# SpaceLearner/SessionRec-pytorch

Hardware: AMD Instinct MI355X
Metric: sessions/sec training, Yoochoose-1/64 batch 512 (higher is better)
Workload: dtype bf16 (MFMA operands; fp32 accumulate, master weights, scoring); 1 GPU; MSGIFSR training step, synthetic Yoochoose-1/64 shape (V=37484 items, d=256, batch 512 per GPU, session length<=20, order 3, dropout 0.1); global_batch=512, parallelism=single GPU

## Files before the change

include/srec.h:

```cpp
#ifndef SREC_H
#define SREC_H
#include "srec_hg.h"

#ifdef __cplusplus
extern "C" {
#endif

#define SREC_BAD_ARG 1001

int srec_gemm_f32(const float* A, int a_rs, int a_cs, const float* B, int b_rs, int b_cs, float* C, int ldc,
                  const float* bias, int M, int N, int K, const int* dyn, int dyn_mode, float alpha, float beta,
                  float* ws, long ws_floats, void* stream);

int srec_gemm_bf16_nt(const float* A, int lda, const float* B, int ldb, float* C, int ldc, const float* bias, int M,
                      int N, int K, const int* dyn, float alpha, float beta, float* ws, long ws_floats, void* stream);

int srec_gemm_bf16_tn(const float* A, int lda, const float* B, int ldb, float* C, int ldc, int Mred, int N, int K,
                      const int* dyn, float alpha, float beta, float* ws, long ws_floats, void* stream);

int srec_ce_plan(int B, int V, int d, int* n_item_tiles, int* n_ranges);
int srec_score_ce_fwd(const float* sr, int ld_sr, const float* E, int ld_e, const float* cs, const int* labels,
                      int B, int V, int d, const int* dynB, float* ws_stats, float* lab_logit, float* lse,
                      float* lossvec, float* loss, void* stream);
int srec_score_ce_bwd(const float* sr, int ld_sr, const float* E, int ld_e, const float* cs, const int* labels,
// ... 173 lines not shown
                          const float* part, const int* cptr, int u_cap, int n_part, void* stream);
int srec_adam_rows_multi(float* W, const float* G, float* M, float* V, int n, int d, int ld, const float* hyper, int use_wd,
                         float max_norm, int renorm_write, float* cs_out, float cs_scale, int eps_mode, float cs_eps,
                         const float* proj_cs, float proj_inv_scale, float* radial, void* dst16, int Dp, int* slot,
                         const float* part, const int* cptr, int u_cap, int n_part, const void* desc, const float* multi_hyper,
                         void* stream);

int srec_hg_ws_floats(const void* desc, long* n_floats);
int srec_hg_fwd(const void* desc, const float* x, int ld_x, float* out, int ld_out, unsigned char* arg, void* stream);
int srec_hg_fold(const void* desc, void* stream);
int srec_step_prep(const void* desc, void* stream);
int srec_hg_drop_prep(const float* x, const float* cnt, int rows, int D, float p, int seed, const int* counter, int salt,
                      float* ms, float* xc, float* rm, float* xres, float pa, long na, float* mk, void* stream);
int srec_hg_drop_prep16(const float* x, const float* cnt, int rows, int D, float p, int seed, const int* counter, int salt,
                        float* ms, float* xc, float* rm, float* xres, float pa, long na, float* mk, void* xc16, void* stream);
int srec_hg_drop_merge(const float* t, int S, const float* ms, long n, float* dx, float p, int seed, const int* counter,
                       int salt, void* stream);
int srec_hg_pre_merge(const void* desc, const float* g, int ld_g, const float* t, int S, float* dx, int ld_dx, void* stream);
int srec_hg_bwd(const void* desc, const float* x, int ld_x, const float* g, int ld_g, const unsigned char* arg, float* dx,
                int ld_dx, float* ws, void* stream);

int srec_gemm_group_bf16(const void* desc, int mode, void* stream);

int srec_gemm_f32_group_run(const void* desc, float* ws, long ws_floats, void* stream);
int srec_gemm_f32_group_run_defer(const void* desc, float* ws, long ws_floats, long* slab_off, int* slab_n, void* stream);
int srec_gemm16_nt(const void* desc, void* stream);
int srec_gemm16_tn(const void* desc, void* stream);
int srec_rows_bf16(const float* src, int ld, int n, const int* dyn, int d, void* dst16, void* stream);
int srec_sum_slabs(const float* part, int C, int R, long n, float* out, void* stream);
int srec_weights_bf16(int n, const void* W, const void* W16, const void* WT16, const int* R, const int* Cc, void* stream);
int srec_norm_perm_pick_fwd(const float* x, int ld_x, const int* perm, int n_cap, const int* dyn_t, int D, int eps_mode,
                            float eps, float* allf, float* invr, int npick, int B, const int* dyn_b, const void* pick,
                            const void* pout, const int* ld_p, void* stream);
int srec_norm_perm_pick_bwd(const float* allf, const float* invr, const float* g_allf, int ld_g, const int* perm, int n_cap,
                            const int* cat_seg, int B, const int* dyn_b, int D, int npick, const void* pick, const void* g_pick,
                            const int* ld_gp, float* dx, int ld_dx, int nt, const int* row0, const int* ncap, const void* dyn_n,
                            int n_rows, void* stream);
int srec_gru_step_fwd(const void* desc, void* stream);
int srec_gru_step_bwd(const void* desc, void* stream);
int srec_gru_fused_fwd(const void* desc, void* stream);
int srec_gru_wfrag(int n, const void* W, const void* dst, int d, void* stream);
// ... 64 lines not shown
```

sessionrec-pytorch_amd/csrc/gemm16.hip:

```cpp
#include "common.h"
#include "../../include/srec_hg.h"

namespace {

typedef __bf16 bf16x8 __attribute__((ext_vector_type(8)));
typedef short short2_t __attribute__((ext_vector_type(2)));
constexpr int G16_MAXP = 16, G16_MAXS = 4;

struct G16Args {
    const unsigned short* A[G16_MAXP][G16_MAXS];
    const unsigned short* B[G16_MAXP][G16_MAXS];
    void* C[G16_MAXP];
    const int* dyn[G16_MAXP];
    int M[G16_MAXP], N[G16_MAXP], K[G16_MAXP], nseg[G16_MAXP], koff[G16_MAXP], nsplit[G16_MAXP], start[G16_MAXP + 1];
    int np, lda, ldb, ldc;
    int ldap[G16_MAXP], ldbp[G16_MAXP], ldcp[G16_MAXP];
    float beta;
    int keep_dead;
    int per_xcd;
    int xcd_gs;
};

__device__ __forceinline__ unsigned lds_addr(const void* p) {
    return (unsigned)(size_t)(__attribute__((address_space(3))) const void*)p;
}

__device__ __forceinline__ void glds16(const unsigned short* sbase, unsigned voff, unsigned lds_dst) {
    unsigned keep;
// ... 21 lines not shown
    else if (PDV >= 3 && ahead >= 2) wait_vm<2 * IPS>();
    else if (PDV >= 2 && ahead >= 1) wait_vm<IPS>();
    else wait_vm<0>();
}

#ifdef SREC_G16_TIMING
__device__ unsigned long long g_g16_tim[8];
__device__ unsigned long long g_g16_blk[8192][2];
#define G16T(i) do { __builtin_amdgcn_sched_barrier(0); g16t[i] = __builtin_readcyclecounter(); __builtin_amdgcn_sched_barrier(0); } while (0)
#else
#define G16T(i)
#endif

constexpr int NS = 4, PD = 3;

template <int TM, int TN, bool C16, int BK = 32, int NS = 4, int NW = 4>
__global__ __launch_bounds__(64 * NW) void gemm16_nt_kernel(G16Args g) {
    constexpr int WN = NW / 2, NT = 64 * NW;
    constexpr int PD = NS - 1;
    constexpr int RPI = 512 / BK;
    constexpr int PPR = BK / 8;
    constexpr int FS = BK == 32 ? 2 : 1;
    constexpr int IM = TM / 64, IN = TN / (32 * WN);
    constexpr int STG = (TM + TN) * BK;
    constexpr int NIA = TM / RPI, NI = (TM + TN) / RPI;
    constexpr int IPS = NI / NW;
    static_assert(NI % NW == 0, "every wave must issue the same number of DMA instructions per stage");
    extern __shared__ __attribute__((aligned(16))) unsigned short smem[];

    const int bid = xcd_tile(g);
    if (bid >= g.start[g.np]) return;
#ifdef SREC_G16_TIMING
// ... 16 lines not shown
    unsigned short* __restrict__ C16p = static_cast<unsigned short*>(g.C[p]);
    if (m0 >= Ml) {
        if (!g.keep_dead && (C16 || g.beta == 0.f))
            for (int i = tid; i < TM * TN / 4; i += NT) {
                const int r = m0 + (i * 4) / TN, c = n0 + (i * 4) % TN;
                if (r < M && c + 3 < N) {
                    if (C16) *reinterpret_cast<uint2*>(C16p + (size_t)r * g.ldcp[p] + c) = make_uint2(0u, 0u);
                    else *reinterpret_cast<float4*>(C + (size_t)r * g.ldcp[p] + c) = make_float4(0.f, 0.f, 0.f, 0.f);
                } else if (r < M) {
                    for (int e = 0; e < 4; ++e)
                        if (c + e < N) { if (C16) C16p[(size_t)r * g.ldcp[p] + c + e] = 0; else C[(size_t)r * g.ldcp[p] + c + e] = 0.f; }
                }
            }
        return;
    }

    f32x16 acc[IM][IN];
#pragma unroll
    for (int i = 0; i < IM; ++i)
#pragma unroll
        for (int j = 0; j < IN; ++j)
#pragma unroll
            for (int r = 0; r < 16; ++r) acc[i][j][r] = 0.f;

    const int nk = K / BK, total = nk * g.nseg[p];
    const unsigned lds0 = lds_addr(smem);
    const int rl = lane / PPR, sl = lane % PPR;
    unsigned voff[IPS];
#pragma unroll
    for (int ii = 0; ii < IPS; ++ii) {
        const int i = ii * NW + wave;
        const int r = RPI * (i < NIA ? i : i - NIA) + rl;
        const unsigned pc = (unsigned)((sl ^ ((r >> FS) & (PPR - 1))) * 8);
        voff[ii] = i < NIA ? ((unsigned)min(r, Ml - 1 - m0) * (unsigned)g.ldap[p] + pc) * 2u
                           : ((unsigned)min(r, N - 1 - n0) * (unsigned)g.ldbp[p] + pc) * 2u;
    }
    int is_seg = 0, is_k = 0;
    const unsigned short* Aseg = g.A[p][0] + (size_t)m0 * g.ldap[p];
    const unsigned short* Bseg = g.B[p][0] + (size_t)n0 * g.ldbp[p];
    auto stage = [&](int it) {
        const unsigned dst = lds0 + (unsigned)((it % NS) * STG) * 2u;
#pragma unroll
        for (int ii = 0; ii < IPS; ++ii) {
            const int i = ii * NW + wave;
            glds16((i < NIA ? Aseg : Bseg) + is_k, voff[ii], dst + (unsigned)i * 1024u);
        }
        is_k += BK;
        if (is_k >= K) {
            is_k = 0;
            if (++is_seg < g.nseg[p]) {
                Aseg = g.A[p][is_seg] + (size_t)m0 * g.ldap[p];
                Bseg = g.B[p][is_seg] + (size_t)n0 * g.ldbp[p];
            }
        }
    };

    for (int s = 0; s < PD && s < total; ++s) stage(s);
    G16T(1);
    for (int it = 0; it < total; ++it) {
        G16T(2);
        wait_stage<IPS, PD>(min(total - it - 1, PD - 1));
        __syncthreads();
        G16T(3);
        if (it + PD < total) stage(it + PD);
        G16T(4);
        const unsigned short* As = smem + (it % NS) * STG;
// ... 32 lines not shown
#pragma unroll
        for (int i = 0; i < IM; ++i)
#pragma unroll
            for (int j = 0; j < IN; ++j)
#pragma unroll
                for (int q = 0; q < 4; ++q) {
                    uint2 v;
                    v.x = srec_pack_bf16(acc[i][j][4 * q], acc[i][j][4 * q + 1]);
                    v.y = srec_pack_bf16(acc[i][j][4 * q + 2], acc[i][j][4 * q + 3]);
                    *reinterpret_cast<uint2*>(patch + (i * 32 + l31) * LDP + j * 32 + 8 * q + 4 * half) = v;
                }
        constexpr int PPW = WC / 8;
#pragma unroll
        for (int t = 0; t < WR * PPW / 64; ++t) {
            const int idx = t * 64 + lane, rr = idx / PPW, pc = idx % PPW;
            const int row = m0 + wm * WR + rr, col = n0 + wn * WC + pc * 8;
            if (row >= M || (g.keep_dead && row >= Ml)) continue;
            uint4 v = *reinterpret_cast<const uint4*>(patch + rr * LDP + pc * 8);
            if (row >= Ml) v = make_uint4(0u, 0u, 0u, 0u);
            if (col + 7 < N) {
                *reinterpret_cast<uint4*>(C16p + (size_t)row * g.ldcp[p] + col) = v;
            } else {
                const unsigned short* e = reinterpret_cast<const unsigned short*>(&v);
                for (int k = 0; k < 8; ++k)
                    if (col + k < N) C16p[(size_t)row * g.ldcp[p] + col + k] = e[k];
            }
        }
#ifdef SREC_G16_TIMING
        asm volatile("s_waitcnt vmcnt(0)" ::: "memory");
        G16T(7);
        if (threadIdx.x == 0 && bid < 8192) g_g16_blk[bid][1] = __builtin_amdgcn_s_memrealtime();
        if (threadIdx.x == 0 && bid == 17) { g_g16_tim[0] = g16t[1] - g16t[0]; g_g16_tim[1] = g16w; g_g16_tim[2] = g16d; g_g16_tim[3] = g16c; g_g16_tim[4] = g16t[7] - g16t[6]; g_g16_tim[5] = g16t[7] - g16t[0]; g_g16_tim[6] = total; }
#endif
        return;
// ... 261 lines not shown
        }
        g.start[p] = blocks;
        blocks += cdiv(d->M[p], tm) * cdiv(d->N[p], tn) * g.nsplit[p];
    }
    g.start[d->np] = blocks;
    return 0;
}

template <typename K>
int optin(K kernel, int bytes, std::atomic<unsigned long long>& done) {
    return bytes > 64 * 1024 ? srec_lds_optin((const void*)kernel, bytes, done) : 0;
}

}

extern "C" int srec_gemm16_nt(const void* desc_, void* stream) {
    const srec_gemm16_group* h = (const srec_gemm16_group*)desc_;
    if (h == nullptr || h->np <= 0 || h->np > G16_MAXP) return SREC_BAD_ARG;
    G16Args g{};
    int blocks = 0;
    auto Mh = [&](int p) { return (h->mhint[p] > 0 && h->mhint[p] < h->M[p]) ? h->mhint[p] : h->M[p]; };
    long t128 = 0, rows_cap = 0, rows_live = 0;
    for (int p = 0; p < h->np; ++p) { t128 += (long)cdiv(Mh(p), 128) * cdiv(h->N[p], 128); rows_cap += h->M[p]; rows_live += Mh(p); }
    int nmax = 0;
    for (int p = 0; p < h->np; ++p) nmax = h->N[p] > nmax ? h->N[p] : nmax;
    int tm = (t128 >= 384 && nmax > 256) ? 128 : 64;
    long t64x128 = 0;
    for (int p = 0; p < h->np; ++p) t64x128 += (long)cdiv(Mh(p), 64) * cdiv(h->N[p], 128);
    if (!(h->c16 & SREC_G16_C_BF16) && tm == 64 && t64x128 > 384) {
        const long r64 = cdiv((int)cdiv((int)t64x128, 8), 96), r128 = cdiv((int)cdiv((int)t128, 8), 64);
        if (r128 * 105 < r64 * 100 || (r128 <= r64 && t128 >= 256)) tm = 128;
    }
    const int tn = (tm == 64 && t64x128 < 192) ? 64 : 128;
    if (int rc = fill(g, desc_, tm, tn, false, blocks)) return rc;
    if (!(h->c16 & SREC_G16_C_BF16)) {
        bool same_tn = true;
        const int tn0 = cdiv(h->N[0], tn);
        for (int p = 1; p < h->np; ++p) same_tn = same_tn && cdiv(h->N[p], tn) == tn0;
        if (same_tn && rows_live * 10 < rows_cap * 9) {
            g.xcd_gs = tn0;
            blocks = cdiv(blocks, 8 * tn0) * 8 * tn0;
        } else {
            g.per_xcd = cdiv(blocks, 8); blocks = 8 * g.per_xcd;
        }
    }
    hipStream_t st = (hipStream_t)stream;
    const bool c16 = h->c16 & SREC_G16_C_BF16;
    static std::atomic<unsigned long long> optin_mask[8];
#define SREC_G16(TMV, TNV, C16V, BKV, NSV, slot)                                                                       \
    do {                                                                                                               \
        const size_t lds = (size_t)NSV * (TMV + TNV) * BKV * 2;                                                        \
        if (int rc = optin(gemm16_nt_kernel<TMV, TNV, C16V, BKV, NSV>, (int)lds, optin_mask[slot])) return rc;         \
        hipLaunchKernelGGL((gemm16_nt_kernel<TMV, TNV, C16V, BKV, NSV>), dim3(blocks), dim3(256), lds, st, g);         \
    } while (0)
    const bool deep = blocks <= 384;
    if (tn == 64) {
        if (c16) SREC_G16(64, 64, true, 64, 2, 0); else if (deep) SREC_G16(64, 64, false, 64, 4, 1); else SREC_G16(64, 64, false, 64, 2, 2);
    } else if (deep && tm == 64 && !c16) {
        SREC_G16(64, 128, false, 64, 4, 3);
    } else if (tm == 128) {
        if (c16) SREC_G16(128, 128, true, 32, 3, 4); else SREC_G16(128, 128, false, 64, 2, 5);
    } else {
        if (c16) SREC_G16(64, 128, true, 32, 3, 6); else SREC_G16(64, 128, false, 64, 2, 7);
    }
#undef SREC_G16
    SREC_LAUNCH_CHECK();
    return 0;
}

#ifdef SREC_G16_TIMING
extern "C" int srec_g16_timing(unsigned long long* tim8, unsigned long long* blk) {
    if (hipMemcpyFromSymbol(tim8, HIP_SYMBOL(g_g16_tim), sizeof(unsigned long long) * 8) != hipSuccess) return 1;
    return hipMemcpyFromSymbol(blk, HIP_SYMBOL(g_g16_blk), sizeof(unsigned long long) * 16384) == hipSuccess ? 0 : 1;
}
extern "C" int srec_g16_timing_reset() {
    static unsigned long long z[16384];
    return hipMemcpyToSymbol(HIP_SYMBOL(g_g16_blk), z, sizeof(z)) == hipSuccess ? 0 : 1;
}
#endif

extern "C" int srec_gemm16_tn(const void* desc_, void* stream) {
    G16Args g{};
// ... 32 lines not shown
```

sessionrec-pytorch_amd/csrc/hgat.hip:

```cpp
#include "common.h"
#include "../../include/srec_hg.h"

extern "C" int srec_hg_fold(const void* desc, void* stream);

namespace {

constexpr int WPB = 4;
constexpr int MAXDEG = SREC_MAX_DEGREE;
constexpr int MAXH = 8;
constexpr int NCHUNK_C = 32;
constexpr int SEGCAP = 1025;
constexpr int NCHUNK = 16;
constexpr int MAXT = SREC_HG_MAXT, MAXM = SREC_HG_MAXM, MAXB = SREC_HG_MAXB, MAXI = SREC_HG_MAXI;

typedef __bf16 bf16x4_t __attribute__((ext_vector_type(4)));
typedef float f32x4_t __attribute__((ext_vector_type(4)));
__device__ __forceinline__ float4 ld4(const float* p) { return *reinterpret_cast<const float4*>(p); }
__device__ __forceinline__ float4 ld4(const unsigned short* p) {
    const uint2 v = *reinterpret_cast<const uint2*>(p);
    return make_float4(__uint_as_float(v.x << 16), __uint_as_float(v.x & 0xffff0000u), __uint_as_float(v.y << 16),
                       __uint_as_float(v.y & 0xffff0000u));
}
__device__ __forceinline__ float ld1(const float* p) { return *p; }
__device__ __forceinline__ float ld1(const unsigned short* p) { return __uint_as_float((unsigned)*p << 16); }
// ... 1599 lines not shown
            f.jobs[m][f.njob[m]++] = t;
        }
        if (d->n_mods > 0) {
            hipLaunchKernelGGL(hg_colsum_final_kernel, dim3(cdiv(2 * HD, 256), 2 * d->n_mods), dim3(256), 0, st, f);
            DattnArgs q{};
            q.H = H; q.D = D;
            for (int m = 0; m < d->n_mods; ++m) { q.W[m] = d->W[m]; q.Z[m] = d->Z[m]; q.dal[m] = d->d_attn_l[m]; q.dar[m] = d->d_attn_r[m]; }
            hipLaunchKernelGGL(hg_dattn_kernel, dim3(d->n_mods * HD / WPB), dim3(256), 0, st, q);
        }
    }
    SREC_LAUNCH_CHECK();
    return 0;
}

namespace {
__global__ void hg_drop_prep_kernel(const float* __restrict__ x, const float* __restrict__ cnt, long n, int D, long rows,
                                    float p, srec_rng rng, float* __restrict__ ms, float* __restrict__ xc,
                                    float* __restrict__ rm, float* __restrict__ xres, int nb1, float pa, long na,
                                    float* __restrict__ mk, unsigned short* __restrict__ xc16) {
    const unsigned key = srec_rng_key(rng);
    if ((int)blockIdx.x >= nb1) {
        const long j = ((long)((int)blockIdx.x - nb1) * blockDim.x + threadIdx.x) * 4;
        const float sa = 1.f / (1.f - pa);
        for (int e = 0; e < 4; ++e)
            if (j + e < na) mk[j + e] = srec_keep(key ^ 0xA5A5A5A5u, (unsigned)(j + e), pa, sa);
        return;
    }
    const long i = ((long)blockIdx.x * blockDim.x + threadIdx.x) * 4;
    if (i >= n) return;
    const float sc = p > 0.f ? 1.f / (1.f - p) : 1.f;
    const long row = i / D;
    const float c0 = cnt[row], c1 = cnt[rows + row];
    const float4 xv = *reinterpret_cast<const float4*>(x + i);
    float4 m0, m1;
    const unsigned i0 = (unsigned)i, i1 = (unsigned)(n + i);
    m0.x = srec_keep(key, i0, p, sc); m0.y = srec_keep(key, i0 + 1, p, sc); m0.z = srec_keep(key, i0 + 2, p, sc); m0.w = srec_keep(key, i0 + 3, p, sc);
    m1.x = srec_keep(key, i1, p, sc); m1.y = srec_keep(key, i1 + 1, p, sc); m1.z = srec_keep(key, i1 + 2, p, sc); m1.w = srec_keep(key, i1 + 3, p, sc);
    if (ms != nullptr) {
        *reinterpret_cast<float4*>(ms + i) = m0;
        *reinterpret_cast<float4*>(ms + n + i) = m1;
    }
    const float4 x0 = make_float4(xv.x * m0.x, xv.y * m0.y, xv.z * m0.z, xv.w * m0.w);
    const float4 x1 = make_float4(xv.x * m1.x, xv.y * m1.y, xv.z * m1.z, xv.w * m1.w);
// ... 26 lines not shown
        const unsigned key = srec_rng_key(rng);
        const float sc = p > 0.f ? 1.f / (1.f - p) : 1.f;
        const unsigned i0 = (unsigned)i, i1 = (unsigned)(n + i);
        m0.x = srec_keep(key, i0, p, sc); m0.y = srec_keep(key, i0 + 1, p, sc); m0.z = srec_keep(key, i0 + 2, p, sc); m0.w = srec_keep(key, i0 + 3, p, sc);
        m1.x = srec_keep(key, i1, p, sc); m1.y = srec_keep(key, i1 + 1, p, sc); m1.z = srec_keep(key, i1 + 2, p, sc); m1.w = srec_keep(key, i1 + 3, p, sc);
    }
    float4 d = *reinterpret_cast<float4*>(dx + i);
    d.x += a.x * m0.x + b.x * m1.x; d.y += a.y * m0.y + b.y * m1.y; d.z += a.z * m0.z + b.z * m1.z; d.w += a.w * m0.w + b.w * m1.w;
    *reinterpret_cast<float4*>(dx + i) = d;
}

}

static int hg_drop_prep_run(const float* x, const float* cnt, int rows, int D, float p, int seed, const int* counter,
                            int salt, float* ms, float* xc, float* rm, float* xres, float pa, long na, float* mk,
                            unsigned short* xc16, void* stream) {
    if (rows <= 0) return 0;
    if (D <= 0 || (D & 3) || p < 0.f || p >= 1.f || pa < 0.f || pa >= 1.f) return SREC_BAD_ARG;
    const long n = (long)rows * D;
    if (2 * n > 0xffffffffL || na > 0xffffffffL) return SREC_BAD_ARG;
    const int nb1 = (int)((n / 4 + 255) / 256);
    const int nb2 = (pa > 0.f && na > 0 && mk != nullptr) ? (int)(((na + 3) / 4 + 255) / 256) : 0;
    hipLaunchKernelGGL(hg_drop_prep_kernel, dim3((unsigned)(nb1 + nb2)), dim3(256), 0, (hipStream_t)stream, x, cnt, n, D,
                       (long)rows, p, srec_rng{(unsigned)seed, counter, (unsigned)salt, p}, ms, xc, rm, xres, nb1, pa, na, mk, xc16);
    SREC_LAUNCH_CHECK();
    return 0;
}

extern "C" int srec_hg_drop_prep(const float* x, const float* cnt, int rows, int D, float p, int seed, const int* counter,
                                 int salt, float* ms, float* xc, float* rm, float* xres, float pa, long na, float* mk,
                                 void* stream) {
    return hg_drop_prep_run(x, cnt, rows, D, p, seed, counter, salt, ms, xc, rm, xres, pa, na, mk, nullptr, stream);
}
extern "C" int srec_hg_drop_prep16(const float* x, const float* cnt, int rows, int D, float p, int seed, const int* counter,
                                   int salt, float* ms, float* xc, float* rm, float* xres, float pa, long na, float* mk,
                                   void* xc16, void* stream) {
    if (xc16 == nullptr) return SREC_BAD_ARG;
    return hg_drop_prep_run(x, cnt, rows, D, p, seed, counter, salt, ms, xc, rm, xres, pa, na, mk, (unsigned short*)xc16, stream);
}

extern "C" int srec_hg_drop_merge(const float* t, int S, const float* ms, long n, float* dx, float p, int seed,
                                  const int* counter, int salt, void* stream) {
    if (n <= 0) return 0;
    if ((n & 3) || S < 1 || p < 0.f || p >= 1.f || 2 * n > 0xffffffffL) return SREC_BAD_ARG;
    hipLaunchKernelGGL(hg_drop_merge_kernel, dim3((unsigned)((n / 4 + 255) / 256)), dim3(256), 0, (hipStream_t)stream, t, S,
                       ms, n, dx, p, srec_rng{(unsigned)seed, counter, (unsigned)salt, p});
    SREC_LAUNCH_CHECK();
    return 0;
}
```

sessionrec-pytorch_amd/hgat.py:

```python
import ctypes as _ct
from collections import namedtuple

import torch

from . import ops
from ._lib import CONST, lib, ptr, stream
from .ops import GemmProb, HgDesc, _ld, _rows

DropState = namedtuple('DropState', 'xc xres mk ms rng cnt')


class HgPlan:

    def __init__(self, H, D, slope, B, dynB, types, modules, blocks, insts, mod_conv=None, layer_id=0, live=None):
        self.mod_conv = mod_conv if mod_conv is not None else [0] * len(modules)
        self.layer_id, self.live = layer_id, dict(live or {})
        self.H, self.D, self.slope, self.B, self.dynB = H, D, slope, B, dynB
        self.types, self.modules, self.blocks, self.insts, self._fold = types, modules, blocks, insts, None
        assert (len(types) <= CONST['SREC_HG_MAXT'] and len(modules) <= CONST['SREC_HG_MAXM'] and
                len(blocks) <= CONST['SREC_HG_MAXB'] and len(insts) <= CONST['SREC_HG_MAXI'])

    def put_fold(self, small, lay):
        self._fold = (small, lay)

# ... 10 lines not shown
    def projectors(self, cv, t):
        t0, nc = self.types[t][:2]
        return [m for m, (r0, nr, _) in enumerate(self.modules)
                if (cv is None or self.mod_conv[m] == cv) and r0 <= t0 and t0 + nc <= r0 + nr
                and any(bm == m and bt == t for bm, bt in self.blocks)]

    def scratch(self, dev):
        H, ncap = self.H, [tp[1] for tp in self.types]
        sizes = [((nm, b), ncap[t] * H) for b, (m, t) in enumerate(self.blocks) for nm in ('eL', 'eR', 'wL', 'wR')]
        sizes += [((nm, m), 2 * self.D * H) for m in range(max(len(self.modules), len(ncap))) for nm in ('V', 'Z')]
        for i, (m, sb, db, gr) in enumerate(self.insts):
            E = max(gr[4].numel(), 1) * H
            sizes += [(('A', i), E), (('DP', i), E), (('der', i), ncap[self.blocks[db][1]] * H)]
        sizes += [(('smean', t), self.B * self.D) for t in range(len(ncap))]
        sizes.append((('sess', 0), sum(ncap)))
        off, lay = 0, {}
        for key, n in sizes:
            lay[key] = off
            off += n
        return torch.empty(max(off, 1), device=dev, dtype=torch.float32), lay

    def fill(self, d, small, lay, P, dP, params, grads, drop=None):
        if drop is not None:
            for m in range(len(self.modules)):
                d.xin[m] = ptr(drop.xc[self.mod_conv[m]])
            d.xres, d.rm_cnt = ptr(drop.xres), ptr(drop.cnt)
            d.rm_p, d.rm_seed, d.rm_counter, d.rm_salt = drop.rng
            for i in range(len(self.insts)):
                d.Mk[i] = ptr(drop.mk[i]) if drop.mk is not None else None
        d.H, d.D, d.slope, d.B, d.dynB = self.H, self.D, self.slope, self.B, ptr(self.dynB)
        d.p16 = CONST['SREC_HG_P16_BF16'] if P and P[0].dtype == torch.bfloat16 else 0
        d.n_types, d.n_mods, d.n_blocks, d.n_inst = len(self.types), len(self.modules), len(self.blocks), len(self.insts)
        base = small.data_ptr()
        for t, (r0, nc, dyn, seg) in enumerate(self.types):
            d.row0[t], d.ncap[t], d.dyn_n[t], d.seg[t] = r0, nc, ptr(dyn), ptr(seg)
            d.smean[t], d.Z[t] = base + 4 * lay[('smean', t)], base + 4 * lay[('Z', t)]
        for m in range(len(self.modules)):
            W, al, ar, bias = params[4 * m:4 * m + 4]
            d.P[m], d.W[m] = ptr(P[m]) if P else None, ptr(W)
            d.V[m], d.Z[m] = base + 4 * lay[('V', m)], base + 4 * lay[('Z', m)]
            d.attn_l[m], d.attn_r[m], d.bias[m] = ptr(al), ptr(ar), ptr(bias)
            if dP is not None:
                d.dP[m] = ptr(dP[m])
                d.d_attn_l[m], d.d_attn_r[m], d.d_bias[m] = (grads[m][j].data_ptr() for j in range(3))
# ... 24 lines not shown
        for (m, sb, db, gr) in plan.insts:
            t0, nc = plan.types[plan.blocks[db][1]][:2]
            host[plan.mod_conv[m], t0:t0 + nc] += 1.0
        if torch.cuda.is_current_stream_capturing():
            raise RuntimeError('instance counts must be cached by an eager warm-up step before graph capture')
        cnt = _CNT_CACHE[key] = host.to(dev)
    return cnt


def gemm_strategy(mode, D, ldx, n_mods, w_contiguous):
    if mode != 'bf16' or D % 8 or ldx != D or not 0 < n_mods <= 8:
        return 'plain'
    return 'g16' if D % 64 == 0 and w_contiguous else 'grouped'


def _drop_prep(x, plan, drop, strategy):
    (pf, pa), (NT, D), dev, tap = drop, x.shape, x.device, ops.DROP_TAP
    cnt = _inst_counts(plan, NT, dev)
    ms = torch.empty(2, NT, D, device=dev, dtype=torch.float32) if tap is not None else None
    xcs, xres = torch.empty(2, NT, D, device=dev, dtype=torch.float32), torch.empty(NT, D, device=dev)
    sizes = [max(gr[4].numel(), 1) * plan.H for (_, _, _, gr) in plan.insts] if pa > 0 else []
    na = sum(sizes)
    allm = torch.empty(na, device=dev, dtype=torch.float32) if pa > 0 else None
    mk = list(torch.split(allm, sizes)) if pa > 0 else None
    seed, rc = ops.rng_args(dev)
    salt = 101 + 2 * plan.layer_id
    args = (ptr(x), ptr(cnt), NT, D, float(pf), seed, rc, salt, ptr(ms), ptr(xcs), None, ptr(xres), float(pa), na, ptr(allm))
    x16 = torch.empty(2, NT, D, device=dev, dtype=torch.bfloat16) if strategy == 'g16' else None
    if x16 is not None:
        lib.srec_hg_drop_prep16(*args, ptr(x16), stream())
    else:
        lib.srec_hg_drop_prep(*args, stream())
    if tap is not None:
        tap.append(dict(ms=ms.clone(), mk=[m.clone() for m in mk] if mk is not None else None))
    return DropState([xcs[0], xcs[1]], xres, mk, ms, (float(pf), seed, rc, salt), cnt), x16


def _project(xin, x16, plan, params, strategy, dev):
    D, HD, nm = plan.D, plan.H * plan.D, len(plan.modules)
    P = [torch.empty(nr, HD, device=dev, dtype=torch.float32 if strategy == 'plain' else torch.bfloat16)
         for (r0, nr, dyn) in plan.modules]
    if strategy == 'g16':
        w16, wt16 = ops.weights_bf16([params[4 * m] for m in range(nm)])
        xin16 = [x16[cv] for cv in plan.mod_conv] if x16 is not None else [ops.rows_bf16(xin[0])] * nm
        probs = [GemmProb(nc, HD, D, [(xin16[m][t0:t0 + nc], w16[m])], P[m][o:o + nc], dyn_t, mhint=plan.live.get(t0, 0))
                 for m in range(nm) for (o, t0, nc, dyn_t) in plan.pieces(m)]
        for i in range(0, len(probs), ops.G16_MAXP):
            ops.gemm16('nt', probs[i:i + ops.G16_MAXP], D, D, HD, c16=True, keep_dead=True)
        return P, (xin16, wt16)
    if strategy == 'grouped':
        ops.gemm_group(0, [(nr, HD, D, [(xin[m][r0:r0 + nr], params[4 * m])], P[m], dyn)
                           for m, (r0, nr, dyn) in enumerate(plan.modules)], D, D, HD, c16=True)
    else:
        for m, (r0, nr, dyn) in enumerate(plan.modules):
            ops.gemm_nt(xin[m][r0:r0 + nr], _rows(params[4 * m]), P[m], None, dyn, 1 if dyn is not None else 0)
    return P, None


def _backward_graph(ctx, x, g, small, arg, P, params, late_dx):
    plan, nm = ctx.plan, len(ctx.plan.modules)
    cov = [sum(plan.types[bt][1] for bm, bt in plan.blocks if bm == m) for m in range(nm)]
    dP = [torch.empty_like(p) if cov[m] == p.shape[0] else torch.zeros_like(p) for m, p in enumerate(P)]
    grads = [[ops.grad_buf(params[4 * m + 1 + j]).view(-1) for j in range(3)] for m in range(nm)]
    dx = torch.empty(x.shape, device=x.device, dtype=torch.float32)
    flat = [p.reshape(-1) if i % 4 else p for i, p in enumerate(params)]
    desc = plan.fill(HgDesc(), small, ctx.lay, P, dP, flat, grads, ctx.drop)
    desc.p16 |= (CONST['SREC_HG_SKIP_DEAD_DP'] if ctx.strategy == 'g16' else 0) | (CONST['SREC_HG_LATE_DX'] if late_dx else 0)
    n = _ct.c_long()
    lib.srec_hg_ws_floats(_ct.addressof(desc), _ct.addressof(n))
    key = (x.device.index, n.value)
    ws = _HG_WS.get(key)
# ... 62 lines not shown
        ops.gemm_group(2, [(HD, D, nr, [(dP[m], xin[m][r0:r0 + nr])], gWs[m], dyn)
                           for m, (r0, nr, dyn) in enumerate(plan.modules)], HD, D, D, a16=True)
    else:
        for m, (r0, nr, dyn) in enumerate(plan.modules):
            ops.gemm_tn(dP[m], xin[m][r0:r0 + nr], gWs[m], dyn)


class HGATLayer(torch.autograd.Function):

    @staticmethod
    def forward(ctx, x, plan, drop, *params):
        x = _rows(x)
        (NT, D), dev, nm = x.shape, x.device, len(plan.modules)
        strategy = gemm_strategy(ops.PRECISION['matmul'], D, _ld(x), nm, all(params[4 * m].is_contiguous() for m in range(nm)))
        dstate, x16 = None, None
        if drop is not None and (drop[0] > 0 or drop[1] > 0):
            x = x.contiguous()
            dstate, x16 = _drop_prep(x, plan, drop, strategy)
        xin = [dstate.xc[cv] for cv in plan.mod_conv] if dstate is not None else [x] * nm
        P, g16 = _project(xin, x16, plan, params, strategy, dev)
        fold = plan.take_fold()
        small, lay = fold or plan.scratch(dev)
        out = torch.empty(NT, D, device=dev, dtype=torch.float32)
        arg = torch.empty(NT, D, device=dev, dtype=torch.uint8)
        flat = [p.reshape(-1) if i % 4 else p for i, p in enumerate(params)]
        desc = plan.fill(HgDesc(), small, lay, P, None, flat, None, dstate)
        if fold is not None:
            desc.p16 |= CONST['SREC_HG_FOLDED']
        lib.srec_hg_fwd(_ct.addressof(desc), ptr(x), _ld(x), ptr(out), D, ptr(arg), stream())
        ctx.save_for_backward(x, small, arg, *P, *params)
        ctx.plan, ctx.lay, ctx.strategy, ctx.drop, ctx.g16 = plan, lay, strategy, dstate, g16
        ctx.defer, ctx.wparams = ops.defer_scope(), [params[4 * m] for m in range(nm)]
        return out

    @staticmethod
    def backward(ctx, g):
        plan, drop, nm = ctx.plan, ctx.drop, len(ctx.plan.modules)
        x, small, arg, *rest = ctx.saved_tensors
        P, params = rest[:nm], rest[nm:]
        g = _rows(g)
        NT, D = x.shape
        late_dx = drop is not None and drop.ms is None and _ld(g) % 4 == 0
        desc, dP, grads, dx = _backward_graph(ctx, x, g, small, arg, P, params, late_dx)
# ... 14 lines not shown
```

sessionrec-pytorch_amd/ops.py:

```python
import ctypes as _ct
import os
from collections import namedtuple

import torch

from ._lib import CONST, STRUCTS, lib, ptr, ptr_array, stream
from .stepq import StepQueue

HgDesc = STRUCTS['srec_hg_desc']
GemmGroup = STRUCTS['srec_gemm_group']
GemmGroup16 = STRUCTS['srec_gemm16_group']
GemmF32Group = STRUCTS['srec_gemm_f32_group']
GruStepDesc = STRUCTS['srec_gru_step_desc']
GruFusedDesc = STRUCTS['srec_gru_fused_desc']
GruFusedBwdDesc = STRUCTS['srec_gru_fused_bwd_desc']
HeadDesc = STRUCTS['srec_head_desc']
HeadBwdDesc = STRUCTS['srec_head_bwd_desc']
StepPrepDesc = STRUCTS['srec_step_prep_desc']
G16_MAXP, GEMM32_MAXP, GRU_MAXP = CONST['SREC_G16_MAXP'], CONST['SREC_GEMM32_MAXP'], CONST['SREC_GRU_MAXP']
HEAD_MAXH, HEAD_MAXW = CONST['SREC_HEAD_MAXH'], CONST['SREC_HEAD_MAXW']


def _rows(t):
    assert t.dim() == 2 and t.dtype == torch.float32, (t.shape, t.dtype)
# ... 1580 lines not shown
        p, i, o = ctx.bwd_csr
        lib.srec_edge_agg(ptr(g), _ld(g), ptr(p), ptr(i), ptr(o), ptr(coef), N, ptr(ctx.dyn), D, ptr(dx), D, stream())
        return dx, None, None, None, None


def edge_coef(ptr_, idx, ew, n, dyn=None):
    coef = torch.zeros(max(ew.numel(), 1), device=ew.device, dtype=torch.float32)
    lib.srec_edge_coef(ptr(ptr_), ptr(idx), ptr(ew), n, ptr(dyn), ptr(coef), stream())
    return coef


def edge_agg(x, coef, fwd_csr, bwd_csr, dyn=None):
    return EdgeAgg.apply(x, coef, fwd_csr, bwd_csr, dyn)


GemmProb = namedtuple('GemmProb', 'M N K segs C dyn koff nsplit ld mhint', defaults=(0, 1, None, 0))


def gemm_group(mode, probs, lda, ldb, ldc, beta=0.0, a16=False, c16=False):
    g = GemmGroup()
    g.np, g.lda, g.ldb, g.ldc, g.beta, g.a16, g.c16 = len(probs), lda, ldb, ldc, beta, int(a16), int(c16)
    for p, q in enumerate(GemmProb(*q) for q in probs):
        g.M[p], g.N[p], g.K[p], g.nseg[p], g.C[p], g.dyn[p] = q.M, q.N, q.K, len(q.segs), ptr(q.C), ptr(q.dyn)
        for si, (A, B) in enumerate(q.segs):
            g.A[p][si], g.B[p][si] = ptr(A), ptr(B)
    lib.srec_gemm_group_bf16(_ct.addressof(g), mode, stream())


def gemm16_desc(probs, lda, ldb, ldc, beta=0.0, c16=False, keep_dead=False):
    assert 0 < len(probs) <= G16_MAXP
    g = GemmGroup16()
    g.np, g.lda, g.ldb, g.ldc, g.beta = len(probs), lda, ldb, ldc, beta
    g.c16 = (CONST['SREC_G16_C_BF16'] if c16 else 0) | (CONST['SREC_G16_KEEP_DEAD'] if keep_dead else 0)
    for p, q in enumerate(GemmProb(*q) for q in probs):
        g.M[p], g.N[p], g.K[p], g.nseg[p], g.C[p], g.dyn[p] = q.M, q.N, q.K, len(q.segs), ptr(q.C), ptr(q.dyn)
        g.koff[p], g.nsplit[p], g.mhint[p] = q.koff, q.nsplit, int(q.mhint or 0)
        if q.ld is not None:
            g.lda_p[p], g.ldb_p[p], g.ldc_p[p] = q.ld
        for si, (A, B) in enumerate(q.segs):
            g.A[p][si], g.B[p][si] = ptr(A), ptr(B)
    return g


def gemm16(kind, probs, lda, ldb, ldc, beta=0.0, c16=False, keep_dead=False):
    g = gemm16_desc(probs, lda, ldb, ldc, beta, c16, keep_dead)
    (lib.srec_gemm16_nt if kind == 'nt' else lib.srec_gemm16_tn)(_ct.addressof(g), stream())


def rows_bf16(x, dyn=None):
    x = _rows(x)
    n, d = x.shape
    out = torch.empty(n, d, device=x.device, dtype=torch.bfloat16)
    lib.srec_rows_bf16(ptr(x), _ld(x), n, ptr(dyn), d, ptr(out), stream())
    return out


def _weights_bf16_args(ws, transposed=True):
    n = len(ws)
    assert 0 < n <= 8
    dev = ws[0].device
# ... 44 lines not shown
        keep.append((hd, flat))
    box = STEP.take_intake()
    if box is not None:
        q.mailbox, q.M, q.counter, q.box_dst, q.box_cap, q.box_err = box[:6]
    lib.srec_step_prep(_ct.addressof(q), stream())
    for w, a, t in zip(w16, a16 if w16 else (), t16 if w16 else ()):
        _wprep_put('w16', w, (a, t))
    for w, f, b_ in zip(gru, of if gru else (), ob if gru else ()):
        _wprep_put('gru', w, (f, b_))
    for (w, t), b_ in zip(head, hb if head else ()):
        _HEAD_WF_CACHE[(w.data_ptr(), tuple(w.shape), t)] = b_
    if fold is not None:
        plan.put_fold(small, lay)


DROP_TAP = None

from .hgat import HgPlan, HGATLayer, hgat_layer
from .gru import (
    GramCombine, GruOrder, GRUExpand, GRUExpandAll, GRUPointwise, _gru_wfrag_args, expand_path, gram_combine, gru_expand,
    gru_expand_all, gru_expand_fast_ok, gru_fused_bwd_desc, gru_fused_desc, gru_fused_ok, gru_step, gru_step_desc, gru_wfrag,
    gru_wfrag_both)
from .score import (
    BiasArgs, CEWorkspace, MixtureArgs, ScoreCE, ScoreLogProb, ScoreStats, TableBF16, _bf16_dim_ok, _byte_ws, _ce_bwd, _ce_fwd, _logp_cols,
    _bias_args, _mixture_args, _pad_rows, _prepare_sr, catalog_bias, finish_table_grad, score_ce, score_items, score_logp, score_norm, score_rank,
    score_select, score_stats, score_topk, sr16_claim, sr16_written, use_bf16_scoring)
```

Baseline: 697,600 sessions/s.

## Project only live hypergraph rows via compacted row lists in bf16 GEMM

After: 707,900 sessions/s (median of 6 runs). 1.01x the previous value.

```diff
diff --git a/include/srec.h b/include/srec.h
--- a/include/srec.h
+++ b/include/srec.h
@@ -211,6 +211,10 @@
                       float* ms, float* xc, float* rm, float* xres, float pa, long na, float* mk, void* stream);
 int srec_hg_drop_prep16(const float* x, const float* cnt, int rows, int D, float p, int seed, const int* counter, int salt,
                         float* ms, float* xc, float* rm, float* xres, float pa, long na, float* mk, void* xc16, void* stream);
+int srec_hg_live_rows(const void* desc, const void* lists, int* counts, void* stream);
+int srec_hg_drop_prep16_live(const float* x, const float* cnt, int rows, int D, float p, int seed, const int* counter, int salt,
+                             float* ms, float* xc, float* rm, float* xres, float pa, long na, float* mk, void* xc16,
+                             const void* desc, const void* lists, int* counts, void* stream);
 int srec_hg_drop_merge(const float* t, int S, const float* ms, long n, float* dx, float p, int seed, const int* counter,
                        int salt, void* stream);
 int srec_hg_pre_merge(const void* desc, const float* g, int ld_g, const float* t, int S, float* dx, int ld_dx, void* stream);
@@ -222,6 +226,7 @@
 int srec_gemm_f32_group_run(const void* desc, float* ws, long ws_floats, void* stream);
 int srec_gemm_f32_group_run_defer(const void* desc, float* ws, long ws_floats, long* slab_off, int* slab_n, void* stream);
 int srec_gemm16_nt(const void* desc, void* stream);
+int srec_gemm16_nt_rows(const void* desc, const void* rows, void* stream);
 int srec_gemm16_tn(const void* desc, void* stream);
 int srec_rows_bf16(const float* src, int ld, int n, const int* dyn, int d, void* dst16, void* stream);
 int srec_sum_slabs(const float* part, int C, int R, long n, float* out, void* stream);
diff --git a/sessionrec-pytorch_amd/csrc/gemm16.hip b/sessionrec-pytorch_amd/csrc/gemm16.hip
--- a/sessionrec-pytorch_amd/csrc/gemm16.hip
+++ b/sessionrec-pytorch_amd/csrc/gemm16.hip
@@ -12,6 +12,7 @@
     const unsigned short* B[G16_MAXP][G16_MAXS];
     void* C[G16_MAXP];
     const int* dyn[G16_MAXP];
+    const int* rows[G16_MAXP];
     int M[G16_MAXP], N[G16_MAXP], K[G16_MAXP], nseg[G16_MAXP], koff[G16_MAXP], nsplit[G16_MAXP], start[G16_MAXP + 1];
     int np, lda, ldb, ldc;
     int ldap[G16_MAXP], ldbp[G16_MAXP], ldcp[G16_MAXP];
@@ -63,8 +64,10 @@
 
 constexpr int NS = 4, PD = 3;
 
-template <int TM, int TN, bool C16, int BK = 32, int NS = 4, int NW = 4>
+template <int TM, int TN, bool C16, int BK = 32, int NS = 4, int NW = 4, bool RL = false>
 __global__ __launch_bounds__(64 * NW) void gemm16_nt_kernel(G16Args g) {
+    static_assert(!RL || (C16 && TM <= 64 * NW), "row lists: bf16-output launches only, one index per thread");
+    __shared__ int rows_s[RL ? TM : 1];
     constexpr int WN = NW / 2, NT = 64 * NW;
     constexpr int PD = NS - 1;
     constexpr int RPI = 512 / BK;
@@ -111,6 +114,13 @@
             }
         return;
     }
+    if (RL) {
+        if (tid < TM) {
+            const int r = m0 + min(tid, Ml - 1 - m0);
+            rows_s[tid] = g.rows[p] != nullptr ? min(max(g.rows[p][r], 0), M - 1) : r;
+        }
+        __syncthreads();
+    }
 
     f32x16 acc[IM][IN];
 #pragma unroll
@@ -129,11 +139,12 @@
         const int i = ii * NW + wave;
         const int r = RPI * (i < NIA ? i : i - NIA) + rl;
         const unsigned pc = (unsigned)((sl ^ ((r >> FS) & (PPR - 1))) * 8);
-        voff[ii] = i < NIA ? ((unsigned)min(r, Ml - 1 - m0) * (unsigned)g.ldap[p] + pc) * 2u
+        voff[ii] = i < NIA ? ((unsigned)(RL ? rows_s[r] : min(r, Ml - 1 - m0)) * (unsigned)g.ldap[p] + pc) * 2u
                            : ((unsigned)min(r, N - 1 - n0) * (unsigned)g.ldbp[p] + pc) * 2u;
     }
     int is_seg = 0, is_k = 0;
-    const unsigned short* Aseg = g.A[p][0] + (size_t)m0 * g.ldap[p];
+    const size_t a0 = RL ? 0 : (size_t)m0 * g.ldap[p];
+    const unsigned short* Aseg = g.A[p][0] + a0;
     const unsigned short* Bseg = g.B[p][0] + (size_t)n0 * g.ldbp[p];
     auto stage = [&](int it) {
         const unsigned dst = lds0 + (unsigned)((it % NS) * STG) * 2u;
@@ -146,7 +157,7 @@
         if (is_k >= K) {
             is_k = 0;
             if (++is_seg < g.nseg[p]) {
-                Aseg = g.A[p][is_seg] + (size_t)m0 * g.ldap[p];
+                Aseg = g.A[p][is_seg] + a0;
                 Bseg = g.B[p][is_seg] + (size_t)n0 * g.ldbp[p];
             }
         }
@@ -209,10 +220,11 @@
 #pragma unroll
         for (int t = 0; t < WR * PPW / 64; ++t) {
             const int idx = t * 64 + lane, rr = idx / PPW, pc = idx % PPW;
-            const int row = m0 + wm * WR + rr, col = n0 + wn * WC + pc * 8;
-            if (row >= M || (g.keep_dead && row >= Ml)) continue;
+            const int trow = m0 + wm * WR + rr, col = n0 + wn * WC + pc * 8;
+            if (trow >= M || ((RL || g.keep_dead) && trow >= Ml)) continue;
+            const int row = RL ? rows_s[wm * WR + rr] : trow;
             uint4 v = *reinterpret_cast<const uint4*>(patch + rr * LDP + pc * 8);
-            if (row >= Ml) v = make_uint4(0u, 0u, 0u, 0u);
+            if (trow >= Ml) v = make_uint4(0u, 0u, 0u, 0u);
             if (col + 7 < N) {
                 *reinterpret_cast<uint4*>(C16p + (size_t)row * g.ldcp[p] + col) = v;
             } else {
@@ -504,11 +516,20 @@
 
 }
 
-extern "C" int srec_gemm16_nt(const void* desc_, void* stream) {
+static int gemm16_nt_run(const void* desc_, const int* const* rows, void* stream) {
     const srec_gemm16_group* h = (const srec_gemm16_group*)desc_;
     if (h == nullptr || h->np <= 0 || h->np > G16_MAXP) return SREC_BAD_ARG;
     G16Args g{};
     int blocks = 0;
+    bool listed = false;
+    for (int p = 0; rows != nullptr && p < h->np; ++p) {
+        g.rows[p] = rows[p];
+        if (rows[p] == nullptr) continue;
+        listed = true;
+        const long lda = h->lda_p[p] > 0 ? h->lda_p[p] : h->lda;
+        if (h->dyn[p] == nullptr || (long)h->M[p] * lda * 2 > 0xffffffffL) return SREC_BAD_ARG;
+    }
+    if (listed && (h->c16 & (SREC_G16_C_BF16 | SREC_G16_KEEP_DEAD)) != (SREC_G16_C_BF16 | SREC_G16_KEEP_DEAD)) return SREC_BAD_ARG;
     auto Mh = [&](int p) { return (h->mhint[p] > 0 && h->mhint[p] < h->M[p]) ? h->mhint[p] : h->M[p]; };
     long t128 = 0, rows_cap = 0, rows_live = 0;
     for (int p = 0; p < h->np; ++p) { t128 += (long)cdiv(Mh(p), 128) * cdiv(h->N[p], 128); rows_cap += h->M[p]; rows_live += Mh(p); }
@@ -536,15 +557,20 @@
     }
     hipStream_t st = (hipStream_t)stream;
     const bool c16 = h->c16 & SREC_G16_C_BF16;
-    static std::atomic<unsigned long long> optin_mask[8];
-#define SREC_G16(TMV, TNV, C16V, BKV, NSV, slot)                                                                       \
+    static std::atomic<unsigned long long> optin_mask[11];
+#define SREC_G16_RL(TMV, TNV, C16V, BKV, NSV, RLV, slot)                                                               \
     do {                                                                                                               \
         const size_t lds = (size_t)NSV * (TMV + TNV) * BKV * 2;                                                        \
-        if (int rc = optin(gemm16_nt_kernel<TMV, TNV, C16V, BKV, NSV>, (int)lds, optin_mask[slot])) return rc;         \
-        hipLaunchKernelGGL((gemm16_nt_kernel<TMV, TNV, C16V, BKV, NSV>), dim3(blocks), dim3(256), lds, st, g);         \
+        if (int rc = optin(gemm16_nt_kernel<TMV, TNV, C16V, BKV, NSV, 4, RLV>, (int)lds, optin_mask[slot])) return rc; \
+        hipLaunchKernelGGL((gemm16_nt_kernel<TMV, TNV, C16V, BKV, NSV, 4, RLV>), dim3(blocks), dim3(256), lds, st, g); \
     } while (0)
+#define SREC_G16(TMV, TNV, C16V, BKV, NSV, slot) SREC_G16_RL(TMV, TNV, C16V, BKV, NSV, false, slot)
     const bool deep = blocks <= 384;
-    if (tn == 64) {
+    if (listed) {
+        if (tn == 64) SREC_G16_RL(64, 64, true, 64, 2, true, 8);
+        else if (tm == 128) SREC_G16_RL(128, 128, true, 32, 3, true, 9);
+        else SREC_G16_RL(64, 128, true, 32, 3, true, 10);
+    } else if (tn == 64) {
         if (c16) SREC_G16(64, 64, true, 64, 2, 0); else if (deep) SREC_G16(64, 64, false, 64, 4, 1); else SREC_G16(64, 64, false, 64, 2, 2);
     } else if (deep && tm == 64 && !c16) {
         SREC_G16(64, 128, false, 64, 4, 3);
@@ -554,8 +580,15 @@
         if (c16) SREC_G16(64, 128, true, 32, 3, 6); else SREC_G16(64, 128, false, 64, 2, 7);
     }
 #undef SREC_G16
+#undef SREC_G16_RL
     SREC_LAUNCH_CHECK();
     return 0;
+}
+
+extern "C" int srec_gemm16_nt(const void* desc_, void* stream) { return gemm16_nt_run(desc_, nullptr, stream); }
+
+extern "C" int srec_gemm16_nt_rows(const void* desc_, const void* rows, void* stream) {
+    return gemm16_nt_run(desc_, (const int* const*)rows, stream);
 }
 
 #ifdef SREC_G16_TIMING
diff --git a/sessionrec-pytorch_amd/csrc/hgat.hip b/sessionrec-pytorch_amd/csrc/hgat.hip
--- a/sessionrec-pytorch_amd/csrc/hgat.hip
+++ b/sessionrec-pytorch_amd/csrc/hgat.hip
@@ -1637,19 +1637,99 @@
 }
 
 namespace {
-__global__ void hg_drop_prep_kernel(const float* __restrict__ x, const float* __restrict__ cnt, long n, int D, long rows,
+struct LiveArgs {
+    const int* out_ptr[MAXB][4];
+    const int* dyn[MAXB];
+    int* list[MAXB];
+    int* counts;
+    int ncap[MAXB], nsrc[MAXB];
+    int nb;
+};
+
+__device__ __forceinline__ void hg_live_rows_block(const LiveArgs& a, int b) {
+    __shared__ int wsum[4];
+    const int tid = threadIdx.x, lane = tid & 63, wave = tid >> 6;
+    const int n = max(0, dyn_count(a.dyn[b], a.ncap[b]));
+    int* __restrict__ list = a.list[b];
+    int base = 0;
+    for (int r0 = 0; r0 < n; r0 += 1024) {
+        const int u0 = r0 + 4 * tid;
+        bool f[4] = {false, false, false, false};
+        for (int q = 0; q < a.nsrc[b]; ++q) {
+            const int* op = a.out_ptr[b][q];
+            int o[5];
+#pragma unroll
+            for (int k = 0; k < 5; ++k) o[k] = u0 + k <= n ? op[u0 + k] : 0;
+#pragma unroll
+            for (int k = 0; k < 4; ++k) f[k] = f[k] || (u0 + k < n && o[k + 1] > o[k]);
+        }
+        const int cnt = (int)f[0] + (int)f[1] + (int)f[2] + (int)f[3];
+        int inc = cnt;
+#pragma unroll
+        for (int d = 1; d < 64; d <<= 1) {
+            const int v = __shfl_up(inc, d, 64);
+            if (lane >= d) inc += v;
+        }
+        if (lane == 63) wsum[wave] = inc;
+        __syncthreads();
+        int off = base + inc - cnt, tot = 0;
+#pragma unroll
+        for (int w = 0; w < 4; ++w) {
+            if (w < wave) off += wsum[w];
+            tot += wsum[w];
+        }
+#pragma unroll
+        for (int k = 0; k < 4; ++k)
+            if (f[k]) list[off++] = u0 + k;
+        base += tot;
+        __syncthreads();
+    }
+    if (tid == 0) a.counts[b] = base;
+}
+
+__global__ __launch_bounds__(256) void hg_live_rows_kernel(LiveArgs a) { hg_live_rows_block(a, (int)blockIdx.x); }
+
+int hg_live_fill(LiveArgs& a, const srec_hg_desc* d, const void* lists, int* counts) {
+    if (d == nullptr || lists == nullptr || counts == nullptr || d->n_blocks <= 0 || d->n_blocks > MAXB || d->n_inst > MAXI) return SREC_BAD_ARG;
+    a.nb = d->n_blocks; a.counts = counts;
+    for (int b = 0; b < d->n_blocks; ++b) {
+        const int t = d->blk_type[b];
+        if (t < 0 || t >= d->n_types || ((int* const*)lists)[b] == nullptr) return SREC_BAD_ARG;
+        a.list[b] = ((int* const*)lists)[b]; a.ncap[b] = d->ncap[t]; a.dyn[b] = d->dyn_n[t]; a.nsrc[b] = 0;
+    }
+    for (int i = 0; i < d->n_inst; ++i) {
+        const int b = d->inst_sblk[i];
+        if (b < 0 || b >= d->n_blocks || a.nsrc[b] >= 4 || d->out_ptr[i] == nullptr) return SREC_BAD_ARG;
+        a.out_ptr[b][a.nsrc[b]++] = d->out_ptr[i];
+    }
+    return 0;
+}
+}
+
+extern "C" int srec_hg_live_rows(const void* desc, const void* lists, int* counts, void* stream) {
+    LiveArgs a{};
+    if (int rc = hg_live_fill(a, (const srec_hg_desc*)desc, lists, counts)) return rc;
+    hipLaunchKernelGGL(hg_live_rows_kernel, dim3(a.nb), dim3(256), 0, (hipStream_t)stream, a);
+    SREC_LAUNCH_CHECK();
+    return 0;
+}
+
+namespace {
+__global__ __launch_bounds__(256) void hg_drop_prep_kernel(const float* __restrict__ x, const float* __restrict__ cnt, long n, int D, long rows,
                                     float p, srec_rng rng, float* __restrict__ ms, float* __restrict__ xc,
                                     float* __restrict__ rm, float* __restrict__ xres, int nb1, float pa, long na,
-                                    float* __restrict__ mk, unsigned short* __restrict__ xc16) {
+                                    float* __restrict__ mk, unsigned short* __restrict__ xc16, LiveArgs live) {
+    if ((int)blockIdx.x < live.nb) { hg_live_rows_block(live, (int)blockIdx.x); return; }
+    const int bx = (int)blockIdx.x - live.nb;
     const unsigned key = srec_rng_key(rng);
-    if ((int)blockIdx.x >= nb1) {
-        const long j = ((long)((int)blockIdx.x - nb1) * blockDim.x + threadIdx.x) * 4;
+    if (bx >= nb1) {
+        const long j = ((long)(bx - nb1) * blockDim.x + threadIdx.x) * 4;
         const float sa = 1.f / (1.f - pa);
         for (int e = 0; e < 4; ++e)
             if (j + e < na) mk[j + e] = srec_keep(key ^ 0xA5A5A5A5u, (unsigned)(j + e), pa, sa);
         return;
     }
-    const long i = ((long)blockIdx.x * blockDim.x + threadIdx.x) * 4;
+    const long i = ((long)bx * blockDim.x + threadIdx.x) * 4;
     if (i >= n) return;
     const float sc = p > 0.f ? 1.f / (1.f - p) : 1.f;
     const long row = i / D;
@@ -1706,15 +1786,20 @@
 
 static int hg_drop_prep_run(const float* x, const float* cnt, int rows, int D, float p, int seed, const int* counter,
                             int salt, float* ms, float* xc, float* rm, float* xres, float pa, long na, float* mk,
-                            unsigned short* xc16, void* stream) {
+                            unsigned short* xc16, void* stream, const LiveArgs& live = LiveArgs{}) {
+    if (rows <= 0 && live.nb > 0) {
+        hipLaunchKernelGGL(hg_live_rows_kernel, dim3(live.nb), dim3(256), 0, (hipStream_t)stream, live);
+        SREC_LAUNCH_CHECK();
+    }
     if (rows <= 0) return 0;
     if (D <= 0 || (D & 3) || p < 0.f || p >= 1.f || pa < 0.f || pa >= 1.f) return SREC_BAD_ARG;
     const long n = (long)rows * D;
     if (2 * n > 0xffffffffL || na > 0xffffffffL) return SREC_BAD_ARG;
     const int nb1 = (int)((n / 4 + 255) / 256);
     const int nb2 = (pa > 0.f && na > 0 && mk != nullptr) ? (int)(((na + 3) / 4 + 255) / 256) : 0;
-    hipLaunchKernelGGL(hg_drop_prep_kernel, dim3((unsigned)(nb1 + nb2)), dim3(256), 0, (hipStream_t)stream, x, cnt, n, D,
-                       (long)rows, p, srec_rng{(unsigned)seed, counter, (unsigned)salt, p}, ms, xc, rm, xres, nb1, pa, na, mk, xc16);
+    hipLaunchKernelGGL(hg_drop_prep_kernel, dim3((unsigned)(live.nb + nb1 + nb2)), dim3(256), 0, (hipStream_t)stream, x, cnt, n, D,
+                       (long)rows, p, srec_rng{(unsigned)seed, counter, (unsigned)salt, p}, ms, xc, rm, xres, nb1, pa, na, mk, xc16,
+                       live);
     SREC_LAUNCH_CHECK();
     return 0;
 }
@@ -1729,6 +1814,15 @@
                                    void* xc16, void* stream) {
     if (xc16 == nullptr) return SREC_BAD_ARG;
     return hg_drop_prep_run(x, cnt, rows, D, p, seed, counter, salt, ms, xc, rm, xres, pa, na, mk, (unsigned short*)xc16, stream);
+}
+
+extern "C" int srec_hg_drop_prep16_live(const float* x, const float* cnt, int rows, int D, float p, int seed, const int* counter,
+                                        int salt, float* ms, float* xc, float* rm, float* xres, float pa, long na, float* mk,
+                                        void* xc16, const void* desc, const void* lists, int* counts, void* stream) {
+    if (xc16 == nullptr) return SREC_BAD_ARG;
+    LiveArgs live{};
+    if (int rc = hg_live_fill(live, (const srec_hg_desc*)desc, lists, counts)) return rc;
+    return hg_drop_prep_run(x, cnt, rows, D, p, seed, counter, salt, ms, xc, rm, xres, pa, na, mk, (unsigned short*)xc16, stream, live);
 }
 
 extern "C" int srec_hg_drop_merge(const float* t, int S, const float* ms, long n, float* dx, float p, int seed,
diff --git a/sessionrec-pytorch_amd/hgat.py b/sessionrec-pytorch_amd/hgat.py
--- a/sessionrec-pytorch_amd/hgat.py
+++ b/sessionrec-pytorch_amd/hgat.py
@@ -4,7 +4,7 @@
 import torch
 
 from . import ops
-from ._lib import CONST, lib, ptr, stream
+from ._lib import CONST, lib, ptr, ptr_array, stream
 from .ops import GemmProb, HgDesc, _ld, _rows
 
 DropState = namedtuple('DropState', 'xc xres mk ms rng cnt')
@@ -48,20 +48,30 @@
             sizes += [(('A', i), E), (('DP', i), E), (('der', i), ncap[self.blocks[db][1]] * H)]
         sizes += [(('smean', t), self.B * self.D) for t in range(len(ncap))]
         sizes.append((('sess', 0), sum(ncap)))
+        sizes += [(('live', b), max(ncap[t], 1)) for b, (m, t) in enumerate(self.blocks)]
+        sizes.append((('nlive', 0), max(len(self.blocks), 1)))
         off, lay = 0, {}
         for key, n in sizes:
             lay[key] = off
             off += n
         return torch.empty(max(off, 1), device=dev, dtype=torch.float32), lay
 
+    def live_rows(self, small, lay):
+        i32 = small.view(torch.int32)
+        lists = [i32[lay[('live', b)]:][:max(self.types[t][1], 1)] for b, (m, t) in enumerate(self.blocks)]
+        return lists, i32[lay[('nlive', 0)]:][:len(self.blocks)]
+
+    def fill_drop(self, d, drop):
+        for m in range(len(self.modules)):
+            d.xin[m] = ptr(drop.xc[self.mod_conv[m]])
+        d.xres, d.rm_cnt = ptr(drop.xres), ptr(drop.cnt)
+        d.rm_p, d.rm_seed, d.rm_counter, d.rm_salt = drop.rng
+        for i in range(len(self.insts)):
+            d.Mk[i] = ptr(drop.mk[i]) if drop.mk is not None else None
+
     def fill(self, d, small, lay, P, dP, params, grads, drop=None):
         if drop is not None:
-            for m in range(len(self.modules)):
-                d.xin[m] = ptr(drop.xc[self.mod_conv[m]])
-            d.xres, d.rm_cnt = ptr(drop.xres), ptr(drop.cnt)
-            d.rm_p, d.rm_seed, d.rm_counter, d.rm_salt = drop.rng
-            for i in range(len(self.insts)):
-                d.Mk[i] = ptr(drop.mk[i]) if drop.mk is not None else None
+            self.fill_drop(d, drop)
         d.H, d.D, d.slope, d.B, d.dynB = self.H, self.D, self.slope, self.B, ptr(self.dynB)
         d.p16 = CONST['SREC_HG_P16_BF16'] if P and P[0].dtype == torch.bfloat16 else 0
         d.n_types, d.n_mods, d.n_blocks, d.n_inst = len(self.types), len(self.modules), len(self.blocks), len(self.insts)
@@ -116,7 +126,7 @@
     return 'g16' if D % 64 == 0 and w_contiguous else 'grouped'
 
 
-def _drop_prep(x, plan, drop, strategy):
+def _drop_prep(x, plan, drop, strategy, live=None):
     (pf, pa), (NT, D), dev, tap = drop, x.shape, x.device, ops.DROP_TAP
     cnt = _inst_counts(plan, NT, dev)
     ms = torch.empty(2, NT, D, device=dev, dtype=torch.float32) if tap is not None else None
@@ -129,7 +139,10 @@
     salt = 101 + 2 * plan.layer_id
     args = (ptr(x), ptr(cnt), NT, D, float(pf), seed, rc, salt, ptr(ms), ptr(xcs), None, ptr(xres), float(pa), na, ptr(allm))
     x16 = torch.empty(2, NT, D, device=dev, dtype=torch.bfloat16) if strategy == 'g16' else None
-    if x16 is not None:
+    if x16 is not None and live is not None:
+        la = ptr_array(live[1])
+        lib.srec_hg_drop_prep16_live(*args, ptr(x16), _ct.addressof(live[0]), _ct.addressof(la), ptr(live[2]), stream())
+    elif x16 is not None:
         lib.srec_hg_drop_prep16(*args, ptr(x16), stream())
     else:
         lib.srec_hg_drop_prep(*args, stream())
@@ -138,25 +151,31 @@
     return DropState([xcs[0], xcs[1]], xres, mk, ms, (float(pf), seed, rc, salt), cnt), x16
 
 
-def _project(xin, x16, plan, params, strategy, dev):
+def _project(xin, x16, plan, params, strategy, P, live=None):
     D, HD, nm = plan.D, plan.H * plan.D, len(plan.modules)
-    P = [torch.empty(nr, HD, device=dev, dtype=torch.float32 if strategy == 'plain' else torch.bfloat16)
-         for (r0, nr, dyn) in plan.modules]
     if strategy == 'g16':
         w16, wt16 = ops.weights_bf16([params[4 * m] for m in range(nm)])
         xin16 = [x16[cv] for cv in plan.mod_conv] if x16 is not None else [ops.rows_bf16(xin[0])] * nm
-        probs = [GemmProb(nc, HD, D, [(xin16[m][t0:t0 + nc], w16[m])], P[m][o:o + nc], dyn_t, mhint=plan.live.get(t0, 0))
-                 for m in range(nm) for (o, t0, nc, dyn_t) in plan.pieces(m)]
+        type_of = {tp[0]: t for t, tp in enumerate(plan.types)}
+        probs = []
+        for m in range(nm):
+            for (o, t0, nc, dyn_t) in plan.pieces(m):
+                rows = None
+                if live is not None and (m, type_of[t0]) in plan.blocks:
+                    b = plan.blocks.index((m, type_of[t0]))
+                    rows, dyn_t = live[0][b], live[1][b:b + 1]
+                probs.append(GemmProb(nc, HD, D, [(xin16[m][t0:t0 + nc], w16[m])], P[m][o:o + nc], dyn_t,
+                                      mhint=plan.live.get(t0, 0), rows=rows))
         for i in range(0, len(probs), ops.G16_MAXP):
             ops.gemm16('nt', probs[i:i + ops.G16_MAXP], D, D, HD, c16=True, keep_dead=True)
-        return P, (xin16, wt16)
+        return xin16, wt16
     if strategy == 'grouped':
         ops.gemm_group(0, [(nr, HD, D, [(xin[m][r0:r0 + nr], params[4 * m])], P[m], dyn)
                            for m, (r0, nr, dyn) in enumerate(plan.modules)], D, D, HD, c16=True)
     else:
         for m, (r0, nr, dyn) in enumerate(plan.modules):
             ops.gemm_nt(xin[m][r0:r0 + nr], _rows(params[4 * m]), P[m], None, dyn, 1 if dyn is not None else 0)
-    return P, None
+    return None
 
 
 def _backward_graph(ctx, x, g, small, arg, P, params, late_dx):
@@ -249,19 +268,27 @@
         (NT, D), dev, nm = x.shape, x.device, len(plan.modules)
         strategy = gemm_strategy(ops.PRECISION['matmul'], D, _ld(x), nm, all(params[4 * m].is_contiguous() for m in range(nm)))
         dstate, x16 = None, None
-        if drop is not None and (drop[0] > 0 or drop[1] > 0):
-            x = x.contiguous()
-            dstate, x16 = _drop_prep(x, plan, drop, strategy)
-        xin = [dstate.xc[cv] for cv in plan.mod_conv] if dstate is not None else [x] * nm
-        P, g16 = _project(xin, x16, plan, params, strategy, dev)
         fold = plan.take_fold()
         small, lay = fold or plan.scratch(dev)
+        P = [torch.empty(nr, plan.H * D, device=dev, dtype=torch.float32 if strategy == 'plain' else torch.bfloat16)
+             for (r0, nr, dyn) in plan.modules]
+        flat = [p.reshape(-1) if i % 4 else p for i, p in enumerate(params)]
+        desc = plan.fill(HgDesc(), small, lay, P, None, flat, None, None)
+        if fold is not None:
+            desc.p16 |= CONST['SREC_HG_FOLDED']
+        live = plan.live_rows(small, lay) if strategy == 'g16' and ops.HG_LIVE_ROWS and plan.blocks else None
+        dropping = drop is not None and (drop[0] > 0 or drop[1] > 0)
+        if dropping:
+            x = x.contiguous()
+            dstate, x16 = _drop_prep(x, plan, drop, strategy, (desc,) + live if live is not None else None)
+            plan.fill_drop(desc, dstate)
+        elif live is not None:
+            la = ptr_array(live[0])
+            lib.srec_hg_live_rows(_ct.addressof(desc), _ct.addressof(la), ptr(live[1]), stream())
+        xin = [dstate.xc[cv] for cv in plan.mod_conv] if dstate is not None else [x] * nm
+        g16 = _project(xin, x16, plan, params, strategy, P, live)
         out = torch.empty(NT, D, device=dev, dtype=torch.float32)
         arg = torch.empty(NT, D, device=dev, dtype=torch.uint8)
-        flat = [p.reshape(-1) if i % 4 else p for i, p in enumerate(params)]
-        desc = plan.fill(HgDesc(), small, lay, P, None, flat, None, dstate)
-        if fold is not None:
-            desc.p16 |= CONST['SREC_HG_FOLDED']
         lib.srec_hg_fwd(_ct.addressof(desc), ptr(x), _ld(x), ptr(out), D, ptr(arg), stream())
         ctx.save_for_backward(x, small, arg, *P, *params)
         ctx.plan, ctx.lay, ctx.strategy, ctx.drop, ctx.g16 = plan, lay, strategy, dstate, g16
diff --git a/sessionrec-pytorch_amd/ops.py b/sessionrec-pytorch_amd/ops.py
--- a/sessionrec-pytorch_amd/ops.py
+++ b/sessionrec-pytorch_amd/ops.py
@@ -1618,7 +1618,7 @@
     return EdgeAgg.apply(x, coef, fwd_csr, bwd_csr, dyn)
 
 
-GemmProb = namedtuple('GemmProb', 'M N K segs C dyn koff nsplit ld mhint', defaults=(0, 1, None, 0))
+GemmProb = namedtuple('GemmProb', 'M N K segs C dyn koff nsplit ld mhint rows', defaults=(0, 1, None, 0, None))
 
 
 def gemm_group(mode, probs, lda, ldb, ldc, beta=0.0, a16=False, c16=False):
@@ -1648,6 +1648,12 @@
 
 def gemm16(kind, probs, lda, ldb, ldc, beta=0.0, c16=False, keep_dead=False):
     g = gemm16_desc(probs, lda, ldb, ldc, beta, c16, keep_dead)
+    rows = [GemmProb(*q).rows for q in probs]
+    if any(r is not None for r in rows):
+        assert kind == 'nt', 'row lists: nt launches only'
+        ra = ptr_array(rows)
+        lib.srec_gemm16_nt_rows(_ct.addressof(g), _ct.addressof(ra), stream())
+        return
     (lib.srec_gemm16_nt if kind == 'nt' else lib.srec_gemm16_tn)(_ct.addressof(g), stream())
 
 
@@ -1722,6 +1728,7 @@
         plan.put_fold(small, lay)
 
 
+HG_LIVE_ROWS = os.environ.get('SREC_HG_LIVE_ROWS', '1') != '0'
 DROP_TAP = None
 
 from .hgat import HgPlan, HGATLayer, hgat_layer
```
